# DallinClark/RealTimeRaytracer

Measured on AMD Instinct MI355X. Metric: Mrays/sec at 1920x1080 1spp (all rays: primary + shadow), higher is better.
Workload: dtype f32

## Files before the change

realtimeraytracer_amd/csrc/kernels/rtr_kernels.hip:

```cpp
#include "rtr_kernels.h"

#include <algorithm>
#include <cstdlib>
#include <cstring>

namespace rtrdev {

constexpr int kBlock = 256;

template <bool STATS, int STACK>
struct InlinePolicy {
    static constexpr bool kShade = true;
    __device__ __forceinline__ void slots_at(uint32_t) {}
    const DeviceScene& sc; int32_t* stack; LocalStats& st;
    __device__ __forceinline__ bool occluded(rtr_v3 o, rtr_v3 d, float tmax, rtr_v3, bool) {
        HitRec h;
        return trace<true, STATS, kBlock>(sc, stack, o, d, 0.001f, tmax, h, st);
    }
};

__device__ __forceinline__ uint32_t wave_sum_u32(uint32_t v) {
#pragma unroll
    for (int o = 32; o > 0; o >>= 1) v += __shfl_xor(v, o);
    return v;
// ... 321 lines not shown
    uint32_t seed0;
    bool parked;
    __device__ __forceinline__ void draw(uint32_t ns) const {
        if (!parked) return;
        for (uint32_t s = 0; s < ns; ++s) {
            const SamplePair r = light_sample_pair(s + seed0);
            pairs[2u * s * BLOCK] = __float_as_uint(r.r1); pairs[(2u * s + 1u) * BLOCK] = __float_as_uint(r.r2);
        }
    }
    __device__ __forceinline__ SamplePair pair(uint32_t s) const {
        if (parked) return SamplePair{__uint_as_float(pairs[2u * s * BLOCK]), __uint_as_float(pairs[(2u * s + 1u) * BLOCK])};
        return light_sample_pair(s + seed0);
    }
};

constexpr uint32_t kGenBlock = 1024;
__global__ __launch_bounds__(kGenBlock) void k_shadow_gen(DeviceScene sc, FrameBatch fb, const float4* hitTuvp,
                                                          const uint32_t* hitCustom, RayQueue queue, uint32_t* count, uint32_t planeStride) {
    __shared__ uint32_t s_off[kGenBlock / 64], s_tot[kGenBlock / 64], s_base;
    __shared__ uint32_t s_pairs[2u * kParkedPairs * kGenBlock];
    uint32_t q;
    const uint32_t frame = batch_frame(blockIdx.x * kGenBlock + threadIdx.x, planeStride, q);
    const RenderArgs& ra = fb.ra[frame < fb.n ? frame : 0u];
    const size_t plane0 = (size_t)frame * ra.spp;
    const uint32_t wave = threadIdx.x >> 6;
    uint32_t px = 0, lrow = 0, py = 0;
    const bool live = frame < fb.n && pixel_of(ra, q, px, lrow, py);
    LocalStats st;
    Accum acc = zero_accum();
    const bool single = ra.spp == 1u;
    Surface sf0;
    bool surf0 = false;
    uint32_t n = 0;
    const ParkedSamples<kGenBlock> smp{(lds_column)&s_pairs[threadIdx.x], light_sample_seed0(px, py, ra.info.frame), ra.numShadowRays <= kParkedPairs};
    if (live) {
        CountPolicy cp{0};
        smp.draw(ra.numShadowRays);
        for (uint32_t i = 0; i < ra.spp; ++i) {
            const size_t k = (plane0 + i) * planeStride + q;
            const float4 r = hitTuvp[k];
            HitRec h; h.t = r.x; h.u = r.y; h.v = r.z; h.prim = __float_as_uint(r.w); h.custom = hitCustom[k];
            Surface sf;
            const bool surf = fetch_surface<false, false>(sc, ra, h, primary_dir(ra, px, py, i), false, acc, sf, st);
            if (surf) light_loops_from<CountPolicy, false>(sc, ra, smp, sf, 0u, acc, cp, st);
            if (i == 0) { sf0 = sf; surf0 = surf; }
        }
        n = cp.n;
    }
    const uint32_t total = wave_sum(n);
    if ((threadIdx.x & 63u) == 0) { s_tot[wave] = total; s_off[wave] = 0; }
    __syncthreads();
    if (threadIdx.x == 0) {
        uint32_t t = 0;
        for (uint32_t w = 0; w < kGenBlock / 64; ++w) t += s_tot[w];
        s_base = t ? atomicAdd(count, t) : 0u;
    }
    __syncthreads();
    uint32_t base = s_base;
    for (uint32_t w = 0; w < wave; ++w) base += s_tot[w];
    if (!live || n == 0) return;
    for (uint32_t i = 0; i < ra.spp; ++i) {
        const size_t k = (plane0 + i) * planeStride + q;
        EmitPolicy pol{queue, (EmitPolicy::lds_word)&s_off[wave], base, (uint32_t)k};
        if (single) {
            if (surf0) { queue_store_origin(queue, k, sf0.hitPoint, sf0.hitNormal); light_loops_from<EmitPolicy, false>(sc, ra, smp, sf0, 0u, acc, pol, st); }
        } else {
            const float4 r = hitTuvp[k];
            HitRec h; h.t = r.x; h.u = r.y; h.v = r.z; h.prim = __float_as_uint(r.w); h.custom = hitCustom[k];
            Surface sf;
            if (fetch_surface<false, false>(sc, ra, h, primary_dir(ra, px, py, i), false, acc, sf, st)) {
                queue_store_origin(queue, k, sf.hitPoint, sf.hitNormal);
                light_loops_from<EmitPolicy, false>(sc, ra, smp, sf, 0u, acc, pol, st);
            }
        }
    }
}

constexpr size_t kBinnedMinRays = (size_t)10 << 20;
constexpr uint32_t kBinnedMinNodes = 1u << 16;
#ifndef RTR_GEN_OCT_BLOCK
#define RTR_GEN_OCT_BLOCK 512
#endif
constexpr uint32_t kGenOctBlock = RTR_GEN_OCT_BLOCK;
constexpr uint32_t kParkSurface = 6, kParkWords = kParkSurface + 2u * kParkedPairs;
#ifndef RTR_GEN_OCT_WAVES
#define RTR_GEN_OCT_WAVES 7
#endif
template <bool SINGLE>
__global__ __launch_bounds__(kGenOctBlock) __attribute__((amdgpu_waves_per_eu(SINGLE ? 8 : RTR_GEN_OCT_WAVES, 8)))
void k_shadow_gen_oct(DeviceScene sc, FrameBatch fb, const float4* hitTuvp, const uint32_t* hitCustom,
                      RayQueue queue, uint32_t* ctrl, uint32_t planeStride, uint2* lists,
                      uint32_t listStride, uint32_t kBatch, uint32_t nt) {
    constexpr uint32_t kWaves = kGenOctBlock / 64;
    __shared__ uint32_t s_tot[kWaves][8], s_run[kWaves][8];
    __shared__ uint32_t s_park[kParkWords * kGenOctBlock];
    uint32_t q;
    const uint32_t frame = batch_frame(blockIdx.x * kGenOctBlock + threadIdx.x, planeStride, q);
    const RenderArgs& ra = fb.ra[frame < fb.n ? frame : 0u];
    const uint32_t spp = SINGLE ? 1u : ra.spp;
    const size_t plane0 = (size_t)frame * spp;
    const uint32_t wave = threadIdx.x >> 6;
    uint32_t px = 0, lrow = 0, py = 0;
    const bool live = frame < fb.n && pixel_of(ra, q, px, lrow, py);
    LocalStats st;
    Accum acc = zero_accum();
    constexpr bool single = SINGLE;
    const lds_column park = (lds_column)&s_park[threadIdx.x];
    const ParkedSamples<kGenOctBlock> smp{park + kParkSurface * kGenOctBlock, light_sample_seed0(px, py, ra.info.frame), ra.numShadowRays <= kParkedPairs};
    CountOctPolicy cp{0ull, 0ull};
    if (live) {
        smp.draw(ra.numShadowRays);
        for (uint32_t i = 0; i < spp; ++i) {
            const size_t k = (plane0 + i) * planeStride + q;
            const float4 r = hitTuvp[k];
            HitRec h; h.t = r.x; h.u = r.y; h.v = r.z; h.prim = __float_as_uint(r.w); h.custom = hitCustom[k];
            Surface sf;
            bool surf = fetch_surface<false, false>(sc, ra, h, primary_dir(ra, px, py, i), false, acc, sf, st);
#if RTR_EXP_DOUBLE_FETCH_GEN
            if (surf) {
                HitRec h2 = h; h2.u = h.u + sf.hitPoint.x * (float)(ra.spp - 1u) * 1.0e-30f; h2.v = h.v + sf.hitNormal.y * (float)(ra.spp - 1u) * 1.0e-30f;
                h2.prim = h.prim + (__float_as_uint(sf.hitPoint.z) == 0x7fc12345u ? 1u : 0u);
                Surface sf2;
                if (fetch_surface<false, false>(sc, ra, h2, primary_dir(ra, px, py, i), false, acc, sf2, st)) sf = sf2;
            }
#endif
            if (surf) {
                if (single) {
                    park[0u * kGenOctBlock] = __float_as_uint(sf.hitPoint.x); park[1u * kGenOctBlock] = __float_as_uint(sf.hitPoint.y); park[2u * kGenOctBlock] = __float_as_uint(sf.hitPoint.z);
                    park[3u * kGenOctBlock] = __float_as_uint(sf.hitNormal.x); park[4u * kGenOctBlock] = __float_as_uint(sf.hitNormal.y); park[5u * kGenOctBlock] = __float_as_uint(sf.hitNormal.z);
                }
                light_loops_from<CountOctPolicy, false>(sc, ra, smp, sf, 0u, acc, cp, st);
            }
        }
    }
    uint32_t mine = 0;
#pragma unroll
    for (uint32_t o = 0; o < 8; ++o) {
        const uint32_t c = (uint32_t)(((o < 4 ? cp.lo : cp.hi) >> ((o & 3u) * 16u)) & 0xffffull);
        mine += c;
        const uint32_t t = wave_total(c);
        if ((threadIdx.x & 63u) == 0) s_tot[wave][o] = t;
    }
    __syncthreads();
    if (threadIdx.x < kQueueLists) {
        const uint32_t o = threadIdx.x / kQueueRegions, x = threadIdx.x % kQueueRegions;
        uint32_t before = 0, len = 0, total = 0;
        uint32_t tot[8] = {0u, 0u, 0u, 0u, 0u, 0u, 0u, 0u};
#pragma unroll
        for (uint32_t w0 = 0; w0 < kWaves; w0 += 4u) {
#pragma unroll
            for (uint32_t w = w0; w < w0 + 4u && w < kWaves; ++w) {
#pragma unroll
                for (uint32_t oo = 0; oo < 8; ++oo) tot[oo] += s_tot[w][oo];
            }
            asm volatile("" : "+v"(tot[0]), "+v"(tot[1]), "+v"(tot[2]), "+v"(tot[3]), "+v"(tot[4]), "+v"(tot[5]), "+v"(tot[6]), "+v"(tot[7]) : : "memory");
        }
#pragma unroll
        for (uint32_t oo = 0; oo < 8; ++oo) {
            before += oo < o ? tot[oo] : 0u;
            len = oo == o ? tot[oo] : len;
            total += tot[oo];
        }
        const uint32_t kB = (kBatch >= 512u && blockIdx.x * 8u >= gridDim.x * 7u) ? kBatch / 2u : kBatch;
        const uint32_t nb = (len + kB - 1) / kB;
        const uint32_t b0 = (x + kQueueRegions - blockIdx.x % kQueueRegions) % kQueueRegions;
        const uint32_t cnt = b0 < nb ? (nb - b0 + kQueueRegions - 1) / kQueueRegions : 0u;
        uint32_t at = 0, pos = 0;
        if (threadIdx.x == 0 && total) at = atomicAdd(ctrl, total);
        if (cnt) pos = atomicAdd(ctrl + kQueueListLens + threadIdx.x, cnt);
        const uint32_t first = (uint32_t)__builtin_amdgcn_readfirstlane((int)at) + before;
        if (x == 0) {
            uint32_t c = first;
            for (uint32_t w = 0; w < kWaves; ++w) { s_run[w][o] = c; c += s_tot[w][o]; }
        }
        for (uint32_t j = 0; j < cnt; ++j) {
            const uint32_t f = (b0 + j * kQueueRegions) * kB;
            lists[(size_t)threadIdx.x * listStride + pos + j] = make_uint2(first + f, len - f < kB ? len - f : kB);
        }
    }
    __syncthreads();
    if (mine == 0) return;
    for (uint32_t i = 0; i < spp; ++i) {
        const size_t k = (plane0 + i) * planeStride + q;
        EmitOctPolicy pol{queue, (EmitOctPolicy::lds_word)&s_run[wave][0], (uint32_t)k, nt};
        if constexpr (single) {
            Surface sf0 = {};
            sf0.hitPoint = rtr_mk(__uint_as_float(park[0u * kGenOctBlock]), __uint_as_float(park[1u * kGenOctBlock]), __uint_as_float(park[2u * kGenOctBlock]));
            sf0.hitNormal = rtr_mk(__uint_as_float(park[3u * kGenOctBlock]), __uint_as_float(park[4u * kGenOctBlock]), __uint_as_float(park[5u * kGenOctBlock]));
            queue_store_origin(queue, k, sf0.hitPoint, sf0.hitNormal);
            light_loops_from<EmitOctPolicy, false>(sc, ra, smp, sf0, 0u, acc, pol, st);
        } else {
            const float4 r = hitTuvp[k];
            HitRec h; h.t = r.x; h.u = r.y; h.v = r.z; h.prim = __float_as_uint(r.w); h.custom = hitCustom[k];
            Surface sf;
            if (fetch_surface<false, false>(sc, ra, h, primary_dir(ra, px, py, i), false, acc, sf, st)) {
                queue_store_origin(queue, k, sf.hitPoint, sf.hitNormal);
                light_loops_from<EmitOctPolicy, false>(sc, ra, smp, sf, 0u, acc, pol, st);
            }
        }
    }
}

#ifndef RTR_REFILL_LDS
#define RTR_REFILL_LDS 1
#endif
#ifndef RTR_LIST_SHARE
#define RTR_LIST_SHARE 1
#endif
constexpr int kTailBlocks = 64;
constexpr int32_t kDone = (int32_t)0x80000000;
constexpr int32_t kAbandoned = (int32_t)0x80000001;
constexpr uint32_t kBatchDefault = 256, kBatchLong = 512;
constexpr size_t kBatchLongQueue = (size_t)100 << 20;

constexpr uint32_t kResNone = 3u;
#ifndef RTR_TRACE_BLOCK
#define RTR_TRACE_BLOCK 256
#endif
constexpr int kTraceBlock = RTR_TRACE_BLOCK;
#ifndef RTR_TRI_AUX
#define RTR_TRI_AUX 0
#endif
#ifndef RTR_NODE_AUX
#define RTR_NODE_AUX 0
#endif
#ifndef RTR_SHADOW_STACK
#define RTR_SHADOW_STACK RTR_WIDE_STACK
#endif
#ifndef RTR_TRACE_TOP
#define RTR_TRACE_TOP 40
#endif
constexpr uint32_t kTopNodes = (uint32_t)RTR_TRACE_TOP * (RTR_TRACE_BLOCK / 256);

template <int STACK>
__global__ __launch_bounds__(kBlock) void k_shadow_trace(DeviceScene sc, const RayQueue queue,
                                                              const uint32_t* __restrict__ count, uint32_t* nextBatch,
                                                              uint8_t* __restrict__ vis, uint32_t visFill, uint32_t kBatch, uint32_t kRefill,
                                                              uint32_t kInnerMin, uint32_t* overflow, uint32_t overflowCap) {
    __shared__ int32_t s_stack[(STACK + 1) * kBlock];
    int32_t* lds = s_stack + threadIdx.x;
    lds[0] = kDone;
    const uint32_t n = *count;
    uint32_t batchPos = 0, batchEnd = 0;
    bool exhausted = false;
    const uint32_t regionLen = ((n + kQueueRegions - 1) / kQueueRegions + kBatch - 1) / kBatch * kBatch;
    const uint32_t myRegion = blockIdx.x % kQueueRegions;
    uint32_t regionTry = 0;
    int32_t cur = kDone;
    int sp = 0;
    rtr_v3 o = rtr_mk(0, 0, 0), d = rtr_mk(0, 0, 0), ga = rtr_mk(0, 0, 0), gb = rtr_mk(0, 0, 0);
    float tmax = 0.f;
    uint32_t slot = 0, rayIndex = 0, res = kResNone, occ = 0;
    const float tmin = 0.001f;
    typedef uint32_t u32x4 __attribute__((ext_vector_type(4)));
    const __amdgpu_buffer_rsrc_t nodeBuf = __builtin_amdgcn_make_buffer_rsrc((void*)sc.nodes, 0, 0xffffffff, 0x00020000);
    const __amdgpu_buffer_rsrc_t triBuf = __builtin_amdgcn_make_buffer_rsrc((void*)sc.tris, 0, 0xffffffff, 0x00020000);

    for (;;) {
        const unsigned long long idle = __ballot(cur == kDone);
        const uint32_t nIdle = (uint32_t)__popcll(idle);
        if (nIdle >= kRefill || nIdle == 64u) {
            if (cur == kDone && res != kResNone) {
                if (res == 2u) { const uint32_t at = atomicAdd(overflow, 1u); if (at < overflowCap) overflow[1u + at] = rayIndex; }
                else { if (res != visFill) vis[slot] = (uint8_t)res; occ += res; }
                res = kResNone;
            }
            if (!exhausted) {
                if (batchPos == batchEnd) {
                    for (;;) {
                        if (regionTry >= kQueueRegions) { exhausted = true; break; }
                        const uint32_t r = (myRegion + regionTry) % kQueueRegions;
                        const uint32_t lo = r * regionLen;
                        uint32_t hi = lo + regionLen; if (hi > n) hi = n;
                        uint32_t b = hi;
                        if (lo < hi) {
                            uint32_t got = 0;
                            if ((threadIdx.x & 63u) == 0) got = atomicAdd(nextBatch + 16u * r, kBatch);
                            got = (uint32_t)__builtin_amdgcn_readfirstlane((int)got);
                            b = got < regionLen ? lo + got : hi;
                        }
                        if (b < hi) { batchPos = b; batchEnd = (b + kBatch < hi) ? b + kBatch : hi; break; }
                        ++regionTry;
                    }
// ... 985 lines not shown
Tunables tunables_from_env() {
    Tunables t;
    for (const TunableField& f : kTunables) {
        char env[64] = "RTR_"; size_t n = 4;
        for (const char* c = f.name; *c && n + 1 < sizeof env; ++c) env[n++] = (char)(*c >= 'a' && *c <= 'z' ? *c - 32 : *c);
        env[n] = 0;
        const char* v = getenv(env);
        if (!v || !*v) continue;
        char* end = nullptr;
        const unsigned long x = strtoul(v, &end, 10);
        if (end == v) continue;
        t.*(f.field) = x < f.lo ? f.lo : (x > f.hi ? f.hi : (uint32_t)x);
    }
    return t;
}

static uint32_t padded_pixels(const RenderArgs& ra) {
    const uint32_t band8 = (ra.localRows + 7u) / 8u;
    return band8 * ra.tilesPerRow * 64u;
}

template <int STACK>
static hipError_t mega_t(const DeviceScene& sc, const RenderArgs& ra, const FrameOut& fo, Counters* stats, hipStream_t s) {
    const uint32_t blocks = (padded_pixels(ra) + kBlock - 1) / kBlock;
    if (stats) hipLaunchKernelGGL((k_megakernel<STACK, true>), dim3(blocks), dim3(kBlock), 0, s, sc, ra, fo, stats);
    else hipLaunchKernelGGL((k_megakernel<STACK, false>), dim3(blocks), dim3(kBlock), 0, s, sc, ra, fo, stats);
    return hipGetLastError();
}

hipError_t launch_megakernel(const DeviceScene& sc, const RenderArgs& ra, const FrameOut& fo, int stackEntries,
                             Counters* stats, hipStream_t stream) {
    switch (stackEntries) {
        case 16: return mega_t<16>(sc, ra, fo, stats, stream);
        case 32: return mega_t<32>(sc, ra, fo, stats, stream);
        case 64: return mega_t<64>(sc, ra, fo, stats, stream);
        default: return hipErrorInvalidValue;
    }
}

template <int STACK>
static hipError_t wave_t(const DeviceScene& sc, const FrameBatch& fb, const Workspace& ws, const Tunables& tun,
                         Counters* stats, hipStream_t s, hipEvent_t* ev, uint32_t numCus) {
    const RenderArgs& ra = fb.ra[0];
    const uint32_t nb = fb.n;
    const uint32_t blocks = (padded_pixels(ra) + kBlock - 1) / kBlock;
    {
        const uint32_t planeVec = (uint32_t)(ws.visPlaneBytes / 16u), pitchVec = ws.rayQueue.slotStride / 16u;
        uint32_t fblocks = std::min<uint32_t>((planeVec + kBlock - 1) / kBlock, std::max<uint32_t>(4096u / std::max<uint32_t>(ws.visPlanes, 1u), 64u));
        if (fblocks == 0) fblocks = 1;
        hipLaunchKernelGGL(k_fill_planes, dim3(fblocks, ws.visPlanes ? ws.visPlanes : 1u), dim3(kBlock), 0, s, reinterpret_cast<uint4*>(ws.vis), ws.visFill * 0x01010101u, planeVec, pitchVec,
                           ws.queueCount, kQueueCtrlWords, ws.overflow);
    }
    if (ev) hipEventRecord(ev[0], s);
    const uint32_t kPersist = tun.primary_persist;
    const uint32_t kPersistMinRays = tun.primary_persist_min_rays;
    const uint32_t kPBatch = tun.primary_batch, kPRefill = tun.primary_refill, kPInnerMin = tun.primary_inner_min, kPWgsPerCu = tun.primary_wgs_per_cu;
    const uint32_t planeStride = blocks * kBlock;
    const unsigned long long camRays = (unsigned long long)planeStride * ra.spp;
    bool packet = false;
    if ((kPersist == 1u || (kPersist == 2u && camRays >= kPersistMinRays)) && nb == 1u && camRays < 0xffffffffull) {
        uint32_t pblocks = numCus * kPWgsPerCu;
        const uint32_t pneeded = (uint32_t)(((unsigned long long)planeStride * ra.spp + kBlock - 1) / kBlock);
        if (pblocks > pneeded) pblocks = pneeded;
        if (pblocks == 0) pblocks = 1;
        if (stats) hipLaunchKernelGGL((k_primary_persist<16, true>), dim3(pblocks), dim3(kBlock), 0, s, sc, fb.ra[0], ws.hitTuvp, ws.hitCustom, ws.rayQueue.origin, stats, ws.queueCount + kPrimaryRedoWord, ws.overflow + 1, ws.queueCount + kPrimaryCursors, planeStride, kPBatch, kPRefill, kPInnerMin);
        else hipLaunchKernelGGL((k_primary_persist<16, false>), dim3(pblocks), dim3(kBlock), 0, s, sc, fb.ra[0], ws.hitTuvp, ws.hitCustom, ws.rayQueue.origin, stats, ws.queueCount + kPrimaryRedoWord, ws.overflow + 1, ws.queueCount + kPrimaryCursors, planeStride, kPBatch, kPRefill, kPInnerMin);
    } else if (tun.primary_wide && sc.nodes4) {
        if (stats) hipLaunchKernelGGL((k_primary4<true>), dim3(blocks * ra.spp * nb), dim3(kBlock), 0, s, sc, fb, ws.hitTuvp, ws.hitCustom, ws.rayQueue.origin, stats, ws.queueCount + kPrimaryRedoWord, ws.overflow + 1, blocks);
        else hipLaunchKernelGGL((k_primary4<false>), dim3(blocks * ra.spp * nb), dim3(kBlock), 0, s, sc, fb, ws.hitTuvp, ws.hitCustom, ws.rayQueue.origin, stats, ws.queueCount + kPrimaryRedoWord, ws.overflow + 1, blocks);
    } else if (tun.primary_packet) {
        packet = true;
        if (stats) hipLaunchKernelGGL((k_primary_packet<true>), dim3(blocks * ra.spp * nb), dim3(kBlock), 0, s, sc, fb, ws.hitTuvp, ws.hitCustom, ws.rayQueue.origin, stats, blocks);
        else hipLaunchKernelGGL((k_primary_packet<false>), dim3(blocks * ra.spp * nb), dim3(kBlock), 0, s, sc, fb, ws.hitTuvp, ws.hitCustom, ws.rayQueue.origin, stats, blocks);
    } else if (stats) hipLaunchKernelGGL((k_primary<STACK, true>), dim3(blocks * (kBlock / kPrimBlock) * ra.spp * nb), dim3(kPrimBlock), 0, s, sc, fb, ws.hitTuvp, ws.hitCustom, ws.rayQueue.origin, stats, ws.queueCount + kPrimaryRedoWord, ws.overflow + 1, blocks * (kBlock / kPrimBlock));
    else hipLaunchKernelGGL((k_primary<STACK, false>), dim3(blocks * (kBlock / kPrimBlock) * ra.spp * nb), dim3(kPrimBlock), 0, s, sc, fb, ws.hitTuvp, ws.hitCustom, ws.rayQueue.origin, stats, ws.queueCount + kPrimaryRedoWord, ws.overflow + 1, blocks * (kBlock / kPrimBlock));
    if (!packet) {
        if (stats) hipLaunchKernelGGL(k_primary_tail<true>, dim3(kTailBlocks), dim3(kBlock), 0, s, sc, fb, ws.hitTuvp, ws.hitCustom, ws.rayQueue.origin, ws.queueCount + kPrimaryRedoWord, ws.overflow + 1, ws.spill, planeStride, stats);
        else hipLaunchKernelGGL(k_primary_tail<false>, dim3(kTailBlocks), dim3(kBlock), 0, s, sc, fb, ws.hitTuvp, ws.hitCustom, ws.rayQueue.origin, ws.queueCount + kPrimaryRedoWord, ws.overflow + 1, ws.spill, planeStride, stats);
    }
    if (ev) hipEventRecord(ev[1], s);
    const uint32_t kBatchEnv = tun.trace_batch;
    const uint32_t kBatch = kBatchEnv >= 64u ? kBatchEnv : ((size_t)nb * blocks * kBlock * ra.spp * ra.maxRaysPerSample >= kBatchLongQueue ? kBatchLong : kBatchDefault);
    const uint32_t kWide = tun.trace_bvh4;
    const uint32_t genBlocks = (nb * blocks * kBlock + kGenBlock - 1) / kGenBlock, genOctBlocks = (nb * blocks * kBlock + kGenOctBlock - 1) / kGenOctBlock;
    const uint32_t binMode = tun.trace_binned;
    const size_t maxRaysQ = (size_t)nb * blocks * kBlock * ra.spp * ra.maxRaysPerSample;
    const bool wide = kWide && sc.nodes4;
    const bool binned = wide && ws.batchLists && (size_t)ra.spp * ra.maxRaysPerSample <= 65535u &&
                        (size_t)ws.capRays / kBatch / kQueueRegions + genOctBlocks <= ws.listStride &&
                        (binMode == 1u || (binMode == 2u && maxRaysQ >= kBinnedMinRays && sc.numNodes4 >= kBinnedMinNodes));
    const uint32_t kNtQueue = tun.queue_nt;
    RayQueue rq = ws.rayQueue;
    rq.ownLeaf = (wide && tun.trace_own_leaf) ? 1u : 0u;
    if (binned && ra.spp == 1u) hipLaunchKernelGGL(k_shadow_gen_oct<true>, dim3(genOctBlocks), dim3(kGenOctBlock), 0, s, sc, fb, ws.hitTuvp, ws.hitCustom, rq, ws.queueCount, blocks * kBlock, ws.batchLists, ws.listStride, kBatch, kNtQueue >> 1);
    else if (binned) hipLaunchKernelGGL(k_shadow_gen_oct<false>, dim3(genOctBlocks), dim3(kGenOctBlock), 0, s, sc, fb, ws.hitTuvp, ws.hitCustom, rq, ws.queueCount, blocks * kBlock, ws.batchLists, ws.listStride, kBatch, kNtQueue >> 1);
    else hipLaunchKernelGGL(k_shadow_gen, dim3(genBlocks), dim3(kGenBlock), 0, s, sc, fb, ws.hitTuvp, ws.hitCustom, rq, ws.queueCount, blocks * kBlock);
    if (ev) hipEventRecord(ev[2], s);
    const size_t maxRays = (size_t)nb * blocks * kBlock * ra.spp * ra.maxRaysPerSample;
    const uint32_t kWgsPerCu = tun.trace_wgs_per_cu;
    uint32_t tblocks = numCus * (kWgsPerCu ? kWgsPerCu : (maxRays >= kBinnedMinRays ? 8u : 6u));
    const uint32_t needed = (uint32_t)((maxRays + kBlock - 1) / kBlock);
    if (tblocks > needed) tblocks = needed;
    if (tblocks == 0) tblocks = 1;
    const uint32_t kRefill = tun.trace_refill, kInnerMin = tun.trace_inner_min;
    (void)sizeof(STACK);
    const uint32_t kOct = tun.trace_octant_forms | ((kNtQueue & 1u) << 1);
    const uint32_t kTop = tun.trace_top_nodes < kTopNodes ? tun.trace_top_nodes : kTopNodes;
    const uint32_t top = kTop < sc.numNodes4 ? kTop : sc.numNodes4;
    uint32_t tblocks4 = tblocks * (uint32_t)kBlock / (uint32_t)kTraceBlock;
    if (tblocks4 == 0) tblocks4 = 1;
    if (wide) {
        if (stats) {
            if (binned) hipLaunchKernelGGL((k_shadow_trace4<RTR_SHADOW_STACK, true, true>), dim3(tblocks4), dim3(kTraceBlock), 0, s, sc, ws.rayQueue, ws.queueCount, ws.queueCount + kBatchCursorWord, ws.vis, ws.visFill, kBatch, kRefill, kInnerMin, ws.overflow, ws.overflowCap, kOct, top, ws.batchLists, ws.listStride, stats, ws.clk);
            else hipLaunchKernelGGL((k_shadow_trace4<RTR_SHADOW_STACK, false, true>), dim3(tblocks4), dim3(kTraceBlock), 0, s, sc, ws.rayQueue, ws.queueCount, ws.queueCount + kBatchCursorWord, ws.vis, ws.visFill, kBatch, kRefill, kInnerMin, ws.overflow, ws.overflowCap, kOct, top, ws.batchLists, ws.listStride, stats, ws.clk);
        } else {
            if (binned) hipLaunchKernelGGL((k_shadow_trace4<RTR_SHADOW_STACK, true, false>), dim3(tblocks4), dim3(kTraceBlock), 0, s, sc, ws.rayQueue, ws.queueCount, ws.queueCount + kBatchCursorWord, ws.vis, ws.visFill, kBatch, kRefill, kInnerMin, ws.overflow, ws.overflowCap, kOct, top, ws.batchLists, ws.listStride, stats, ws.clk);
            else hipLaunchKernelGGL((k_shadow_trace4<RTR_SHADOW_STACK, false, false>), dim3(tblocks4), dim3(kTraceBlock), 0, s, sc, ws.rayQueue, ws.queueCount, ws.queueCount + kBatchCursorWord, ws.vis, ws.visFill, kBatch, kRefill, kInnerMin, ws.overflow, ws.overflowCap, kOct, top, ws.batchLists, ws.listStride, stats, ws.clk);
        }
    } else hipLaunchKernelGGL((k_shadow_trace<16>), dim3(tblocks), dim3(kBlock), 0, s, sc, ws.rayQueue, ws.queueCount, ws.queueCount + kBatchCursorWord, ws.vis, ws.visFill, kBatch, kRefill, kInnerMin, ws.overflow, ws.overflowCap);
    if (ev) hipEventRecord(ev[5], s);
    if (stats) hipLaunchKernelGGL((k_shadow_tail<true>), dim3(kTailBlocks), dim3(kBlock), 0, s, sc, ws.rayQueue, ws.overflow, ws.overflowCap, ws.queueCount, ws.vis, ws.spill, stats);
    else hipLaunchKernelGGL((k_shadow_tail<false>), dim3(kTailBlocks), dim3(kBlock), 0, s, sc, ws.rayQueue, ws.overflow, ws.overflowCap, ws.queueCount, ws.vis, ws.spill, stats);
    if (ev) hipEventRecord(ev[3], s);
    const uint32_t kRowWaves = tun.resolve_row_waves;
    const uint32_t rowWaves = (kRowWaves && ra.tilesPerRow % 8u == 0u && blocks % 2u == 0u) ? 1u : 0u;
    const bool full = (ra.images & ~((1u << 1) | (1u << 16))) != 0u;
    const bool compact = !stats && !full && tun.resolve_compact && !rowWaves && ra.numShadowRays >= 1u && ra.numShadowRays <= kResolveMaxSamples &&
                         sc.numLights <= kResolveMaxLights && sc.numLightTris <= kResolveMaxLightTris;
    if (compact) hipLaunchKernelGGL(k_resolve_compact, dim3(blocks * nb), dim3(kBlock), 0, s, sc, fb, blocks * kBlock, ws.hitTuvp, ws.hitCustom, ws.vis, ws.rayQueue.slotStride);
    else if (stats) {
        if (full) hipLaunchKernelGGL((k_resolve<true, true>), dim3(blocks * nb), dim3(kBlock), 0, s, sc, fb, blocks * kBlock, ws.hitTuvp, ws.hitCustom, ws.vis, ws.rayQueue.slotStride, stats, rowWaves);
        else hipLaunchKernelGGL((k_resolve<true, false>), dim3(blocks * nb), dim3(kBlock), 0, s, sc, fb, blocks * kBlock, ws.hitTuvp, ws.hitCustom, ws.vis, ws.rayQueue.slotStride, stats, rowWaves);
    } else {
        if (full) hipLaunchKernelGGL((k_resolve<false, true>), dim3(blocks * nb), dim3(kBlock), 0, s, sc, fb, blocks * kBlock, ws.hitTuvp, ws.hitCustom, ws.vis, ws.rayQueue.slotStride, stats, rowWaves);
        else hipLaunchKernelGGL((k_resolve<false, false>), dim3(blocks * nb), dim3(kBlock), 0, s, sc, fb, blocks * kBlock, ws.hitTuvp, ws.hitCustom, ws.vis, ws.rayQueue.slotStride, stats, rowWaves);
    }
    if (ev) hipEventRecord(ev[4], s);
    return hipGetLastError();
}

hipError_t launch_wavefront(const DeviceScene& sc, const FrameBatch& fb, const Workspace& ws, const Tunables& tun,
                            int stackEntries, Counters* stats, hipStream_t stream, hipEvent_t* ev, uint32_t numCus) {
    if (numCus == 0) numCus = 256;
    if (fb.n < 1 || fb.n > kMaxBatch) return hipErrorInvalidValue;
    switch (stackEntries) {
        case 16: return wave_t<16>(sc, fb, ws, tun, stats, stream, ev, numCus);
        case 32: return wave_t<32>(sc, fb, ws, tun, stats, stream, ev, numCus);
        case 64: return wave_t<64>(sc, fb, ws, tun, stats, stream, ev, numCus);
        default: return hipErrorInvalidValue;
    }
}

hipError_t launch_occlusion_walk(const DeviceScene& sc, const OcclusionArgs& oa, const Tunables& tun, bool alpha, Counters* stats, hipStream_t s, uint32_t numCus,
                                 const RayMaskArgs& rm) {
    if (numCus == 0) numCus = 256;
    if (!sc.nodes4) return hipErrorInvalidValue;
    RayQueue rq;
    rq.dt = const_cast<float4*>(oa.rays); rq.slot = oa.queue;
    const bool hinted = oa.startLeaves != nullptr;
    if (hinted) { rq.origin = reinterpret_cast<float4*>(const_cast<int32_t*>(oa.startLeaves)); rq.slotMask = oa.numTris; }
    uint32_t tblocks = numCus * (tun.trace_wgs_per_cu ? tun.trace_wgs_per_cu : (oa.n >= kBinnedMinRays ? 8u : 6u)) * (uint32_t)kBlock / (uint32_t)kTraceBlock;
    const uint32_t needed = (uint32_t)(((uint64_t)oa.n + kTraceBlock - 1) / kTraceBlock);
    if (tblocks > needed) tblocks = needed;
    if (tblocks == 0) tblocks = 1;
    const uint32_t kOct = tun.trace_octant_forms | ((tun.queue_nt & 1u) << 1) | (alpha ? 0u : 4u);
    const uint32_t kTop = tun.trace_top_nodes < kTopNodes ? tun.trace_top_nodes : kTopNodes;
    const uint32_t top = kTop < sc.numNodes4 ? kTop : sc.numNodes4;
    uint32_t* const ctrl = oa.ctrl;
    const bool masked = rm.masked != 0u;
    if (masked) rq.slotStride = (rm.cullMask & 0xffu) | ((rm.masked & kCullAll) << 4);
    const uint32_t* const cnt = masked ? reinterpret_cast<const uint32_t*>(rm.rayMasks) : ctrl;
#define RTR_OCC_WALK(STATS, HINTS, MASKED) hipLaunchKernelGGL((k_shadow_trace4<RTR_SHADOW_STACK, true, STATS, true, HINTS, MASKED>), dim3(tblocks), dim3(kTraceBlock), 0, s, sc, rq, cnt, ctrl + kBatchCursorWord, \
        oa.occluded, 0u, oa.batch, tun.trace_refill, tun.trace_inner_min, oa.overflow, oa.overflowCap, kOct, top, oa.lists, oa.listStride, stats, (unsigned long long*)nullptr)
    if (masked) {
        if (hinted) { if (stats) RTR_OCC_WALK(true, true, true); else RTR_OCC_WALK(false, true, true); }
        else { if (stats) RTR_OCC_WALK(true, false, true); else RTR_OCC_WALK(false, false, true); }
    } else if (hinted) { if (stats) RTR_OCC_WALK(true, true, false); else RTR_OCC_WALK(false, true, false); }
    else { if (stats) RTR_OCC_WALK(true, false, false); else RTR_OCC_WALK(false, false, false); }
#undef RTR_OCC_WALK
    return hipGetLastError();
}

hipError_t launch_light_tris(const RtrAreaLightInfo* lights, const RtrVertex* vertices, const uint32_t* indices, const uint32_t* first,
                             uint32_t numLights, float4* out, hipStream_t stream) {
    if (numLights == 0) return hipSuccess;
    hipLaunchKernelGGL(k_light_tris, dim3((numLights + 63u) / 64u), dim3(64), 0, stream, lights, vertices, indices, first, numLights, out);
    return hipGetLastError();
}

hipError_t launch_object_terms(const RtrObjectInfo* objects, uint32_t numObjects, float4* out, hipStream_t stream) {
    if (numObjects == 0) return hipSuccess;
    hipLaunchKernelGGL(k_object_terms, dim3((numObjects + 63u) / 64u), dim3(64), 0, stream, objects, numObjects, out);
    return hipGetLastError();
}

hipError_t gen_oct_attributes(bool single, hipFuncAttributes* out) {
    return single ? hipFuncGetAttributes(out, reinterpret_cast<const void*>(&k_shadow_gen_oct<true>))
                  : hipFuncGetAttributes(out, reinterpret_cast<const void*>(&k_shadow_gen_oct<false>));
}

hipError_t launch_deinterleave(const uint32_t* gathered, uint32_t* dst, uint32_t width, uint32_t height,
                               uint32_t bandRows, uint32_t shardCount, uint32_t localRows, hipStream_t stream) {
    const size_t total = (size_t)width * height;
    uint32_t blocks = (uint32_t)((total + kBlock - 1) / kBlock);
    if (blocks > 2048u) blocks = 2048u;
    if (blocks == 0) blocks = 1;
    hipLaunchKernelGGL(k_deinterleave, dim3(blocks), dim3(kBlock), 0, stream, gathered, dst, width, height, bandRows, shardCount, localRows);
    return hipGetLastError();
}

}
```

realtimeraytracer_amd/csrc/rtr_api_render.cpp:

```cpp
#include "../../include/rtr.h"
#include "kernels/rtr_kernels.h"
#include "kernels/rtr_post.h"
#include "rtr_api_internal.h"

#include <hip/hip_runtime.h>

#include <algorithm>
#include <cstdio>
#include <cstring>
#include <vector>

using namespace rtrapi;

struct rtr_frame {
    rtr_ctx* ctx = nullptr;
    uint32_t width = 0, rows = 0, images = 0;
    DevBuf<uint32_t> img[8];
    uint32_t* ext[8] = {nullptr, nullptr, nullptr, nullptr, nullptr, nullptr, nullptr, nullptr};
    DevBuf<float4> hdr;
    DevBuf<float4> hitTuvp, rayDT, rayOrigin;
    DevBuf<uint32_t> raySlot;
    uint32_t slotStride = 0;
    uint32_t visFill = 1;
    DevBuf<uint32_t> hitCustom, queueCount;
// ... 462 lines not shown

int rtr_frame_get_stats(const rtr_frame* f, rtr_frame_stats* out) {
    if (!f || !out) return fail(RTR_ERR_INVALID_ARGUMENT, "rtr_frame_get_stats: null argument");
    *out = f->stats;
    return RTR_OK;
}

static int enqueue_denoise_combine(rtr_frame* f, int iterations, const char* who) {
    if (!f) return fail(RTR_ERR_INVALID_ARGUMENT, "%s: null frame", who);
    if (iterations < 0 || iterations > 64) return fail(RTR_ERR_INVALID_ARGUMENT, "%s: iterations %d", who, iterations);
    for (int i = 0; i < 8; ++i)
        if (!f->image_ptr(i)) return fail(RTR_ERR_INVALID_ARGUMENT, "%s: the frame lacks image %d (create it with all of images 0-7)", who, i);
    HIP_TRY(hipSetDevice(f->ctx->device));
    { const int rc = order_on_own_stream(f); if (rc != RTR_OK) return rc; }
    hipStream_t st = f->ctx->stream;
    uint32_t* sh = f->image_ptr(RTR_IMAGE_SHADOWED); uint32_t* un = f->image_ptr(RTR_IMAGE_UNSHADOWED);
    uint32_t* dsh = f->image_ptr(RTR_IMAGE_DENOISED_SHADOWED); uint32_t* dun = f->image_ptr(RTR_IMAGE_DENOISED_UNSHADOWED);
    const uint32_t* nrm = f->image_ptr(RTR_IMAGE_NORMAL); const uint32_t* pos = f->image_ptr(RTR_IMAGE_POSITION);
    int denoisingOutput = 1;
    for (int i = 0; i < iterations; ++i) {
        const int step = (i + 1) * 1;
        hipError_t e;
        if (denoisingOutput == 1) {
            e = rtrdev::launch_denoise_pair(un, dun, sh, dsh, nrm, pos, f->width, f->rows, step, 1.0f, 0.001f, 0.001f, st);
        } else {
            e = rtrdev::launch_denoise_pair(dun, un, dsh, sh, nrm, pos, f->width, f->rows, step, 1.0f, 0.001f, 0.001f, st);
        }
        if (e != hipSuccess) return fail(RTR_ERR_HIP, "denoise launch: %s", hipGetErrorString(e));
        denoisingOutput = 1 - denoisingOutput;
    }
    hipError_t e = rtrdev::launch_combine(f->image_ptr(RTR_IMAGE_ANALYTIC), denoisingOutput == 0 ? sh : dsh, denoisingOutput == 0 ? un : dun,
                                          f->image_ptr(RTR_IMAGE_FINAL), f->width, f->rows, st);
    if (e != hipSuccess) return fail(RTR_ERR_HIP, "combine launch: %s", hipGetErrorString(e));
    return RTR_OK;
}

int rtr_denoise_combine(rtr_frame* f, int iterations) {
    const int rc = enqueue_denoise_combine(f, iterations, "rtr_denoise_combine");
    if (rc != RTR_OK) return rc;
    HIP_TRY(hipStreamSynchronize(f->ctx->stream));
    return RTR_OK;
}

int rtr_denoise_combine_async(rtr_frame* f, int iterations) {
    return enqueue_denoise_combine(f, iterations, "rtr_denoise_combine_async");
}

int rtr_deinterleave_bands(rtr_ctx* ctx, const void* gathered, void* dst, uint32_t width, uint32_t height, uint32_t bandRows, uint32_t shardCount) {
    if (!ctx || !gathered || !dst || width == 0 || height == 0) return fail(RTR_ERR_INVALID_ARGUMENT, "rtr_deinterleave_bands: bad argument");
    if (bandRows == 0) bandRows = 8;
    if (shardCount == 0) shardCount = 1;
    HIP_TRY(hipSetDevice(ctx->device));
    const uint32_t localRows = rtr_shard_rows(height, bandRows, shardCount);
    hipError_t e = rtrdev::launch_deinterleave((const uint32_t*)gathered, (uint32_t*)dst, width, height, bandRows, shardCount, localRows, ctx->stream);
    if (e != hipSuccess) return fail(RTR_ERR_HIP, "deinterleave launch: %s", hipGetErrorString(e));
    return RTR_OK;
}

int rtr_deinterleave_images(rtr_ctx* ctx, const void* gathered, uint32_t numImages, void* const* dst, uint32_t width, uint32_t height,
                            uint32_t bandRows, uint32_t shardCount) {
    if (!ctx || !gathered || !dst || width == 0 || height == 0) return fail(RTR_ERR_INVALID_ARGUMENT, "rtr_deinterleave_images: bad argument");
    if (numImages == 0 || numImages > rtrdev::kMaxDeinterleaveImages) return fail(RTR_ERR_INVALID_ARGUMENT, "rtr_deinterleave_images: %u images, 1 to %u", numImages, rtrdev::kMaxDeinterleaveImages);
    for (uint32_t i = 0; i < numImages; ++i) if (!dst[i]) return fail(RTR_ERR_INVALID_ARGUMENT, "rtr_deinterleave_images: destination %u is null", i);
    if (bandRows == 0) bandRows = 8;
    if (bandRows % 8u) return fail(RTR_ERR_INVALID_ARGUMENT, "rtr_deinterleave_images: bandRows %u is not a multiple of 8", bandRows);
    if (shardCount == 0) shardCount = 1;
    HIP_TRY(hipSetDevice(ctx->device));
    const uint32_t localRows = rtr_shard_rows(height, bandRows, shardCount);
    uint32_t* d[rtrdev::kMaxDeinterleaveImages];
    for (uint32_t i = 0; i < numImages; ++i) d[i] = static_cast<uint32_t*>(dst[i]);
    hipError_t e = rtrdev::launch_deinterleave_images(static_cast<const uint32_t*>(gathered), d, numImages, width, height, bandRows, shardCount, localRows, ctx->stream);
    if (e != hipSuccess) return fail(RTR_ERR_HIP, "deinterleave launch: %s", hipGetErrorString(e));
    return RTR_OK;
}

#ifdef RTR_TEST_HOOKS
int rtr_test_gen_oct_attributes(int single, uint32_t out[4]) {
    if (!out) return fail(RTR_ERR_INVALID_ARGUMENT, "rtr_test_gen_oct_attributes: null output");
    hipFuncAttributes a{};
    HIP_TRY(rtrdev::gen_oct_attributes(single != 0, &a));
    out[0] = (uint32_t)a.numRegs; out[1] = (uint32_t)a.localSizeBytes; out[2] = (uint32_t)a.sharedSizeBytes; out[3] = (uint32_t)a.maxThreadsPerBlock;
    return RTR_OK;
}
#endif

}
```

Measured before the change: 16880.

## Map each spp sample plane to its own wave in binned shadow generation

The binned shadow-ray generator now assigns one thread per (pixel, sample) instead of looping over samples per thread. The multi-sample variant uses 1024-thread blocks and always parks surfaces in LDS instead of refetching them. The spp-aware binning eligibility check is relaxed accordingly. The spp=1 path keeps its old mapping, so the benchmarked 1spp workload mostly just sees a template rename and forced waves_per_eu of 8.

After: 16900, median of 5. No clear change (+0.1%).

```diff
diff --git a/realtimeraytracer_amd/csrc/kernels/rtr_kernels.hip b/realtimeraytracer_amd/csrc/kernels/rtr_kernels.hip
--- a/realtimeraytracer_amd/csrc/kernels/rtr_kernels.hip
+++ b/realtimeraytracer_amd/csrc/kernels/rtr_kernels.hip
@@ -427,55 +427,55 @@
 #define RTR_GEN_OCT_BLOCK 512
 #endif
 constexpr uint32_t kGenOctBlock = RTR_GEN_OCT_BLOCK;
+constexpr uint32_t kGenOctBlockPlanes = 1024;
 constexpr uint32_t kParkSurface = 6, kParkWords = kParkSurface + 2u * kParkedPairs;
-#ifndef RTR_GEN_OCT_WAVES
-#define RTR_GEN_OCT_WAVES 7
-#endif
-template <bool SINGLE>
-__global__ __launch_bounds__(kGenOctBlock) __attribute__((amdgpu_waves_per_eu(SINGLE ? 8 : RTR_GEN_OCT_WAVES, 8)))
+template <uint32_t BLOCK, bool PLANES>
+__global__ __launch_bounds__(BLOCK) __attribute__((amdgpu_waves_per_eu(8, 8)))
 void k_shadow_gen_oct(DeviceScene sc, FrameBatch fb, const float4* hitTuvp, const uint32_t* hitCustom,
                       RayQueue queue, uint32_t* ctrl, uint32_t planeStride, uint2* lists,
                       uint32_t listStride, uint32_t kBatch, uint32_t nt) {
-    constexpr uint32_t kWaves = kGenOctBlock / 64;
+    constexpr uint32_t kWaves = BLOCK / 64;
     __shared__ uint32_t s_tot[kWaves][8], s_run[kWaves][8];
-    __shared__ uint32_t s_park[kParkWords * kGenOctBlock];
-    uint32_t q;
-    const uint32_t frame = batch_frame(blockIdx.x * kGenOctBlock + threadIdx.x, planeStride, q);
+    __shared__ uint32_t s_park[kParkWords * BLOCK];
+    const uint32_t g = blockIdx.x * BLOCK + threadIdx.x;
+    const uint32_t spp = PLANES ? fb.ra[0].spp : 1u;
+    uint32_t q, frame, sample;
+    if constexpr (!PLANES) { frame = batch_frame(g, planeStride, q); sample = 0u; }
+    else {
+        const uint32_t wv = (uint32_t)__builtin_amdgcn_readfirstlane((int)(g >> 6)), perFrame = spp * (planeStride >> 6);
+        frame = wv / perFrame;
+        const uint32_t r = wv - frame * perFrame, tile = r / spp;
+        sample = r - tile * spp;
+        q = tile * 64u + (threadIdx.x & 63u);
+    }
+    const uint32_t k = (frame * spp + sample) * planeStride + q;
     const RenderArgs& ra = fb.ra[frame < fb.n ? frame : 0u];
-    const uint32_t spp = SINGLE ? 1u : ra.spp;
-    const size_t plane0 = (size_t)frame * spp;
     const uint32_t wave = threadIdx.x >> 6;
     uint32_t px = 0, lrow = 0, py = 0;
     const bool live = frame < fb.n && pixel_of(ra, q, px, lrow, py);
     LocalStats st;
     Accum acc = zero_accum();
-    constexpr bool single = SINGLE;
     const lds_column park = (lds_column)&s_park[threadIdx.x];
-    const ParkedSamples<kGenOctBlock> smp{park + kParkSurface * kGenOctBlock, light_sample_seed0(px, py, ra.info.frame), ra.numShadowRays <= kParkedPairs};
+    const ParkedSamples<BLOCK> smp{park + kParkSurface * BLOCK, light_sample_seed0(px, py, ra.info.frame), ra.numShadowRays <= kParkedPairs};
     CountOctPolicy cp{0ull, 0ull};
     if (live) {
         smp.draw(ra.numShadowRays);
-        for (uint32_t i = 0; i < spp; ++i) {
-            const size_t k = (plane0 + i) * planeStride + q;
-            const float4 r = hitTuvp[k];
-            HitRec h; h.t = r.x; h.u = r.y; h.v = r.z; h.prim = __float_as_uint(r.w); h.custom = hitCustom[k];
-            Surface sf;
-            bool surf = fetch_surface<false, false>(sc, ra, h, primary_dir(ra, px, py, i), false, acc, sf, st);
+        const float4 r = hitTuvp[k];
+        HitRec h; h.t = r.x; h.u = r.y; h.v = r.z; h.prim = __float_as_uint(r.w); h.custom = hitCustom[k];
+        Surface sf;
+        bool surf = fetch_surface<false, false>(sc, ra, h, primary_dir(ra, px, py, sample), false, acc, sf, st);
 #if RTR_EXP_DOUBLE_FETCH_GEN
-            if (surf) {
-                HitRec h2 = h; h2.u = h.u + sf.hitPoint.x * (float)(ra.spp - 1u) * 1.0e-30f; h2.v = h.v + sf.hitNormal.y * (float)(ra.spp - 1u) * 1.0e-30f;
-                h2.prim = h.prim + (__float_as_uint(sf.hitPoint.z) == 0x7fc12345u ? 1u : 0u);
-                Surface sf2;
-                if (fetch_surface<false, false>(sc, ra, h2, primary_dir(ra, px, py, i), false, acc, sf2, st)) sf = sf2;
-            }
-#endif
-            if (surf) {
-                if (single) {
-                    park[0u * kGenOctBlock] = __float_as_uint(sf.hitPoint.x); park[1u * kGenOctBlock] = __float_as_uint(sf.hitPoint.y); park[2u * kGenOctBlock] = __float_as_uint(sf.hitPoint.z);
-                    park[3u * kGenOctBlock] = __float_as_uint(sf.hitNormal.x); park[4u * kGenOctBlock] = __float_as_uint(sf.hitNormal.y); park[5u * kGenOctBlock] = __float_as_uint(sf.hitNormal.z);
-                }
-                light_loops_from<CountOctPolicy, false>(sc, ra, smp, sf, 0u, acc, cp, st);
-            }
+        if (surf) {
+            HitRec h2 = h; h2.u = h.u + sf.hitPoint.x * (float)(ra.spp - 1u) * 1.0e-30f; h2.v = h.v + sf.hitNormal.y * (float)(ra.spp - 1u) * 1.0e-30f;
+            h2.prim = h.prim + (__float_as_uint(sf.hitPoint.z) == 0x7fc12345u ? 1u : 0u);
+            Surface sf2;
+            if (fetch_surface<false, false>(sc, ra, h2, primary_dir(ra, px, py, sample), false, acc, sf2, st)) sf = sf2;
+        }
+#endif
+        if (surf) {
+            park[0u * BLOCK] = __float_as_uint(sf.hitPoint.x); park[1u * BLOCK] = __float_as_uint(sf.hitPoint.y); park[2u * BLOCK] = __float_as_uint(sf.hitPoint.z);
+            park[3u * BLOCK] = __float_as_uint(sf.hitNormal.x); park[4u * BLOCK] = __float_as_uint(sf.hitNormal.y); park[5u * BLOCK] = __float_as_uint(sf.hitNormal.z);
+            light_loops_from<CountOctPolicy, false>(sc, ra, smp, sf, 0u, acc, cp, st);
         }
     }
     uint32_t mine = 0;
@@ -525,25 +525,12 @@
     }
     __syncthreads();
     if (mine == 0) return;
-    for (uint32_t i = 0; i < spp; ++i) {
-        const size_t k = (plane0 + i) * planeStride + q;
-        EmitOctPolicy pol{queue, (EmitOctPolicy::lds_word)&s_run[wave][0], (uint32_t)k, nt};
-        if constexpr (single) {
-            Surface sf0 = {};
-            sf0.hitPoint = rtr_mk(__uint_as_float(park[0u * kGenOctBlock]), __uint_as_float(park[1u * kGenOctBlock]), __uint_as_float(park[2u * kGenOctBlock]));
-            sf0.hitNormal = rtr_mk(__uint_as_float(park[3u * kGenOctBlock]), __uint_as_float(park[4u * kGenOctBlock]), __uint_as_float(park[5u * kGenOctBlock]));
-            queue_store_origin(queue, k, sf0.hitPoint, sf0.hitNormal);
-            light_loops_from<EmitOctPolicy, false>(sc, ra, smp, sf0, 0u, acc, pol, st);
-        } else {
-            const float4 r = hitTuvp[k];
-            HitRec h; h.t = r.x; h.u = r.y; h.v = r.z; h.prim = __float_as_uint(r.w); h.custom = hitCustom[k];
-            Surface sf;
-            if (fetch_surface<false, false>(sc, ra, h, primary_dir(ra, px, py, i), false, acc, sf, st)) {
-                queue_store_origin(queue, k, sf.hitPoint, sf.hitNormal);
-                light_loops_from<EmitOctPolicy, false>(sc, ra, smp, sf, 0u, acc, pol, st);
-            }
-        }
-    }
+    EmitOctPolicy pol{queue, (EmitOctPolicy::lds_word)&s_run[wave][0], k, nt};
+    Surface sf0 = {};
+    sf0.hitPoint = rtr_mk(__uint_as_float(park[0u * BLOCK]), __uint_as_float(park[1u * BLOCK]), __uint_as_float(park[2u * BLOCK]));
+    sf0.hitNormal = rtr_mk(__uint_as_float(park[3u * BLOCK]), __uint_as_float(park[4u * BLOCK]), __uint_as_float(park[5u * BLOCK]));
+    queue_store_origin(queue, k, sf0.hitPoint, sf0.hitNormal);
+    light_loops_from<EmitOctPolicy, false>(sc, ra, smp, sf0, 0u, acc, pol, st);
 }
 
 #ifndef RTR_REFILL_LDS
@@ -1695,18 +1682,19 @@
     const uint32_t kBatchEnv = tun.trace_batch;
     const uint32_t kBatch = kBatchEnv >= 64u ? kBatchEnv : ((size_t)nb * blocks * kBlock * ra.spp * ra.maxRaysPerSample >= kBatchLongQueue ? kBatchLong : kBatchDefault);
     const uint32_t kWide = tun.trace_bvh4;
-    const uint32_t genBlocks = (nb * blocks * kBlock + kGenBlock - 1) / kGenBlock, genOctBlocks = (nb * blocks * kBlock + kGenOctBlock - 1) / kGenOctBlock;
+    const uint32_t genBlocks = (nb * blocks * kBlock + kGenBlock - 1) / kGenBlock, genOctLanes = ra.spp == 1u ? kGenOctBlock : kGenOctBlockPlanes,
+                   genOctBlocks = (nb * ra.spp * blocks * kBlock + genOctLanes - 1) / genOctLanes;
     const uint32_t binMode = tun.trace_binned;
     const size_t maxRaysQ = (size_t)nb * blocks * kBlock * ra.spp * ra.maxRaysPerSample;
     const bool wide = kWide && sc.nodes4;
-    const bool binned = wide && ws.batchLists && (size_t)ra.spp * ra.maxRaysPerSample <= 65535u &&
+    const bool binned = wide && ws.batchLists && ra.maxRaysPerSample <= 65535u &&
                         (size_t)ws.capRays / kBatch / kQueueRegions + genOctBlocks <= ws.listStride &&
                         (binMode == 1u || (binMode == 2u && maxRaysQ >= kBinnedMinRays && sc.numNodes4 >= kBinnedMinNodes));
     const uint32_t kNtQueue = tun.queue_nt;
     RayQueue rq = ws.rayQueue;
     rq.ownLeaf = (wide && tun.trace_own_leaf) ? 1u : 0u;
-    if (binned && ra.spp == 1u) hipLaunchKernelGGL(k_shadow_gen_oct<true>, dim3(genOctBlocks), dim3(kGenOctBlock), 0, s, sc, fb, ws.hitTuvp, ws.hitCustom, rq, ws.queueCount, blocks * kBlock, ws.batchLists, ws.listStride, kBatch, kNtQueue >> 1);
-    else if (binned) hipLaunchKernelGGL(k_shadow_gen_oct<false>, dim3(genOctBlocks), dim3(kGenOctBlock), 0, s, sc, fb, ws.hitTuvp, ws.hitCustom, rq, ws.queueCount, blocks * kBlock, ws.batchLists, ws.listStride, kBatch, kNtQueue >> 1);
+    if (binned && ra.spp == 1u) hipLaunchKernelGGL((k_shadow_gen_oct<kGenOctBlock, false>), dim3(genOctBlocks), dim3(kGenOctBlock), 0, s, sc, fb, ws.hitTuvp, ws.hitCustom, rq, ws.queueCount, blocks * kBlock, ws.batchLists, ws.listStride, kBatch, kNtQueue >> 1);
+    else if (binned) hipLaunchKernelGGL((k_shadow_gen_oct<kGenOctBlockPlanes, true>), dim3(genOctBlocks), dim3(kGenOctBlockPlanes), 0, s, sc, fb, ws.hitTuvp, ws.hitCustom, rq, ws.queueCount, blocks * kBlock, ws.batchLists, ws.listStride, kBatch, kNtQueue >> 1);
     else hipLaunchKernelGGL(k_shadow_gen, dim3(genBlocks), dim3(kGenBlock), 0, s, sc, fb, ws.hitTuvp, ws.hitCustom, rq, ws.queueCount, blocks * kBlock);
     if (ev) hipEventRecord(ev[2], s);
     const size_t maxRays = (size_t)nb * blocks * kBlock * ra.spp * ra.maxRaysPerSample;
@@ -1808,8 +1796,8 @@
 }
 
 hipError_t gen_oct_attributes(bool single, hipFuncAttributes* out) {
-    return single ? hipFuncGetAttributes(out, reinterpret_cast<const void*>(&k_shadow_gen_oct<true>))
-                  : hipFuncGetAttributes(out, reinterpret_cast<const void*>(&k_shadow_gen_oct<false>));
+    return single ? hipFuncGetAttributes(out, reinterpret_cast<const void*>(&k_shadow_gen_oct<kGenOctBlock, false>))
+                  : hipFuncGetAttributes(out, reinterpret_cast<const void*>(&k_shadow_gen_oct<kGenOctBlockPlanes, true>));
 }
 
 hipError_t launch_deinterleave(const uint32_t* gathered, uint32_t* dst, uint32_t width, uint32_t height,
diff --git a/realtimeraytracer_amd/csrc/rtr_api_render.cpp b/realtimeraytracer_amd/csrc/rtr_api_render.cpp
--- a/realtimeraytracer_amd/csrc/rtr_api_render.cpp
+++ b/realtimeraytracer_amd/csrc/rtr_api_render.cpp
@@ -568,6 +568,18 @@
     out[0] = (uint32_t)a.numRegs; out[1] = (uint32_t)a.localSizeBytes; out[2] = (uint32_t)a.sharedSizeBytes; out[3] = (uint32_t)a.maxThreadsPerBlock;
     return RTR_OK;
 }
+
+int rtr_test_frame_queue_route(rtr_frame* f, uint32_t out[3]) {
+    if (!f || !out) return fail(RTR_ERR_INVALID_ARGUMENT, "rtr_test_frame_queue_route: null argument");
+    if (!f->queueCount.p) return fail(RTR_ERR_INVALID_ARGUMENT, "rtr_test_frame_queue_route: the frame has led no staged launch");
+    HIP_TRY(hipSetDevice(f->ctx->device));
+    HIP_TRY(hipStreamSynchronize(f->ctx->stream));
+    uint32_t ctrl[rtrdev::kQueueCtrlWords];
+    HIP_TRY(hipMemcpy(ctrl, f->queueCount.p, sizeof ctrl, hipMemcpyDeviceToHost));
+    out[0] = ctrl[rtrdev::kQueueLenWord]; out[1] = 0; out[2] = f->listStride;
+    for (uint32_t r = 0; r < rtrdev::kQueueLists; ++r) out[1] += ctrl[rtrdev::kQueueListLens + r];
+    return RTR_OK;
+}
 #endif
 
 }
```
